# hyperlogic/splatapult

Measured on AMD Instinct MI355X. Metric: frames_per_sec, higher is better.
Workload: dtype f32; 1 GPU; 1M synthetic Gaussians, SH3, 1920x1080 fp32, 64-step orbit (BASELINE configs[1]); key=cfg2, splats=1000000, width=1920, height=1080, views=1, framebuffer=fp32, frames_in_flight=4, gpu_max_hw_queues=4, async_submit=True, cameras=64-step orbit

## Files before the change

### __graft_entry__.py

```python
import os
import subprocess
import sys

ROOT = os.path.dirname(os.path.abspath(__file__))
LIB = os.path.join(ROOT, "splatapult_amd", "lib", "libmsplat.so")
SOURCES = [os.path.join(ROOT, "splatapult_amd", "csrc", "msplat_device.hip"),
           os.path.join(ROOT, "splatapult_amd", "csrc", "msplat_group.hip"),
           os.path.join(ROOT, "splatapult_amd", "host", "gaussian_scene.cpp"),
           os.path.join(ROOT, "splatapult_amd", "host", "scene_config.cpp"),
           os.path.join(ROOT, "splatapult_amd", "host", "point_scene.cpp")]
HEADERS = [os.path.join(ROOT, "splatapult_amd", "csrc", h) for h in
           ("msplat_kernels.hip.h", "msplat_common.hip.h", "msplat_sort.hip.h", "msplat_cloud.hip.h", "msplat_project.hip.h",
            "msplat_binning.hip.h", "msplat_composite.hip.h", "msplat_points.hip.h", "msplat_occlusion.hip.h",
            "msplat_upload.hip.inc", "msplat_bands.hip.inc", "msplat_getters.hip.inc")] + [
           os.path.join(ROOT, "splatapult_amd", "host", "gaussian_scene.hpp"),
           os.path.join(ROOT, "splatapult_amd", "host", "scene_config.hpp"),
           os.path.join(ROOT, "splatapult_amd", "host", "point_scene.hpp"),
           os.path.join(ROOT, "splatapult_amd", "host", "two_pass_controller.hpp"),
           os.path.join(ROOT, "include", "msplat.h"), os.path.join(ROOT, "include", "msplat_debug.h")]
HIPCC_FLAGS = ["--offload-arch=gfx950", "-O3", "-std=c++17", "-fPIC", "-shared", "-ffp-contract=off",
               "-Wall", "-Wno-unused-function"]


def _stale(target, deps):
    if not os.path.exists(target):
        return True
    t = os.path.getmtime(target)
    return any(os.path.getmtime(d) > t for d in deps if os.path.exists(d))


def build(force=False):
    os.makedirs(os.path.dirname(LIB), exist_ok=True)
    if force or _stale(LIB, SOURCES + HEADERS):
        hipcc = os.environ.get("HIPCC", "/opt/rocm/bin/hipcc")
        cmd = [hipcc] + HIPCC_FLAGS + ["-o", LIB] + SOURCES + ["-lpthread"]
        subprocess.run(cmd, check=True, cwd=ROOT)
    subprocess.run(["make", "-C", os.path.join(ROOT, "oracle")], check=True, stdout=subprocess.DEVNULL)
    if ROOT not in sys.path:
        sys.path.insert(0, ROOT)
    import splatapult_amd
    L = splatapult_amd.lib()
    from splatapult_amd import _capi
    for name, _, _ in _capi.SYMBOLS:
        if os.environ.get("MSPLAT_LIB_PATH") and not hasattr(L, name):
            continue
        getattr(L, name)
# ... 37 lines not shown
```

### include/msplat_debug.h

```cpp
#ifndef MSPLAT_DEBUG_H
#define MSPLAT_DEBUG_H

#include "msplat.h"

#ifdef __cplusplus
extern "C" {
#endif

int msplat_debug_get_projected(msplat_ctx* ctx, float* rec12, uint32_t* rect, uint32_t cap);
int msplat_debug_get_tile_lists(msplat_ctx* ctx, uint32_t* tile_start, uint32_t tile_cap, uint32_t* pairs, uint64_t pair_cap);
int msplat_debug_verify_order(msplat_ctx* ctx, uint32_t* key_violations, uint32_t* list_violations);
int msplat_debug_get_cull_boxes(msplat_ctx* ctx, uint32_t* live, uint32_t* total, int* listed);

int msplat_debug_two_pass(msplat_ctx* ctx, float share, uint64_t* two_pass_frames, float* share_now);
int msplat_get_two_pass_info(msplat_ctx* ctx, uint64_t out[8]);

typedef struct msplat_composite_work {
    uint64_t work_items;
    uint64_t list_entries;
    uint64_t pair_words_fetched;
    uint64_t records_fetched;
    uint64_t records_composited;
    uint64_t pixel_evals;
    uint64_t batches;
    uint64_t clocks_sum, clocks_max, inner_clocks_sum;
    uint64_t useful_evals;
} msplat_composite_work;
int msplat_set_tile_probe(msplat_ctx* ctx, int enable);
int msplat_debug_get_tile_probe8(msplat_ctx* ctx, uint32_t* dst8, uint32_t tile_cap);
int msplat_get_composite_work(msplat_ctx* ctx, msplat_composite_work* out);

int msplat_debug_get_compositor_launch(msplat_ctx* ctx, uint32_t out[4]);

int msplat_debug_band_exchange_loopback(msplat_ctx* ctx, void* comm, int32_t kind, int32_t block_rows, int32_t world, int32_t rank,
                                        const void* src, void* dst, uint64_t pitch_bytes, int32_t width, int32_t height, int32_t flags);

int msplat_debug_cu_partition(msplat_ctx* ctx, uint32_t* mask8);

int msplat_debug_sh_q8_round(const float rec_in[61], float rec_out[61], float steps_out[3], int8_t codes_out[45]);

int msplat_debug_upload_kernel_ms(msplat_ctx* ctx, float* ms);

#ifdef __cplusplus
}
#endif
#endif
```

### splatapult_amd/_capi.py

```python
import ctypes as C
import os

_HERE = os.path.dirname(os.path.abspath(__file__))
LIB_PATH = os.environ.get("MSPLAT_LIB_PATH") or os.path.join(_HERE, "lib", "libmsplat.so")

OK = 0
ERR_INVALID_ARG, ERR_NO_DEVICE, ERR_HIP, ERR_NO_CLOUD, ERR_NO_SORT, ERR_UNSUPPORTED, ERR_PAIR_OVERFLOW, ERR_IO = \
    -1, -2, -3, -4, -5, -6, -7, -8
ERR_PAIR_OVERFLOW_EARLIER = -9
FB_RGBA32F, FB_RGBA16F, FB_RGBA8, FB_SRGB8_ALPHA8 = 0, 1, 2, 3
FB_FORMATS = {"fp32": FB_RGBA32F, "fp16": FB_RGBA16F, "rgba8": FB_RGBA8, "srgb8": FB_SRGB8_ALPHA8}
FB_NAMES = {v: n for n, v in FB_FORMATS.items()}
FB_DTYPES = {FB_RGBA32F: "float32", FB_RGBA16F: "float16", FB_RGBA8: "uint8", FB_SRGB8_ALPHA8: "uint8"}
ROP_NONE, ROP_RGBA8, ROP_RGBA16F = 0, 1, 2
RANK_AUTO, RANK_BALLOT = 0, 1
FRAMES_AUTO, FRAMES_SERIAL, FRAMES_IN_FLIGHT = 0, 1, 2
SPATIAL_AUTO, SPATIAL_ON, SPATIAL_OFF = 0, 1, 2
TWO_PASS_AUTO, TWO_PASS_ON, TWO_PASS_OFF = 0, 1, 2
BANDS_CONTIGUOUS, BANDS_INTERLEAVED, BANDS_BLOCK_INTERLEAVED, BANDS_ROOT_WEIGHTED = 0, 1, 2, 3
EXCHANGE_WIRE_FP16 = 1
CU_ALL, CU_EVEN, CU_ODD = 0, 1, 2
STORAGE_FP32, STORAGE_SH_FP16 = 0, 1
CLOUD_STORAGES = {"fp32": STORAGE_FP32, "sh_fp16": STORAGE_SH_FP16}
STORAGE_SH_Q8 = 3
# ... 112 lines not shown
    ("msplat_points_import_ply", C.c_int, [C.c_void_p, C.c_char_p]),
    ("msplat_points_export_ply", C.c_int, [C.c_void_p, C.c_char_p]),
    ("msplat_points_init_debug", None, [C.c_void_p]),
    ("msplat_points_num", C.c_uint64, [C.c_void_p]),
    ("msplat_points_stride", C.c_uint32, [C.c_void_p]),
    ("msplat_points_data", C.c_void_p, [C.c_void_p]),
    ("msplat_upload_points", C.c_int, [C.c_void_p, C.c_void_p, C.c_uint64, C.c_uint32, C.c_uint32, C.c_uint32]),
    ("msplat_upload_point_cloud", C.c_int, [C.c_void_p, C.c_void_p]),
    ("msplat_set_point_sprite", C.c_int, [C.c_void_p, C.c_void_p, C.c_uint32, C.c_uint32]),
    ("msplat_set_depth_test", C.c_int, [C.c_void_p, C.c_int]),
    ("msplat_set_target_emulation", C.c_int, [C.c_void_p, C.c_int]),
    ("msplat_set_target_mode", C.c_int, [C.c_void_p, C.c_int32]),
    ("msplat_get_target_mode", C.c_int, [C.c_void_p]),
    ("msplat_group_set_target_mode", C.c_int, [C.c_void_p, C.c_int32]),
    ("msplat_attach_cloud", C.c_int, [C.c_void_p, C.c_void_p]),
    ("msplat_stream_wait", C.c_int, [C.c_void_p, C.c_void_p]),
    ("msplat_wait_event", C.c_int, [C.c_void_p, C.c_void_p]),
    ("msplat_sort_count", C.c_int, [C.c_void_p, _U32P]),
    ("msplat_get_sorted_indices", C.c_int, [C.c_void_p, _U32P, C.c_uint32]),
    ("msplat_get_sorted_keys", C.c_int, [C.c_void_p, _U32P, C.c_uint32]),
    ("msplat_get_storage_order", C.c_int, [C.c_void_p, _U32P, C.c_uint64, C.POINTER(C.c_int)]),
    ("msplat_debug_get_cull_boxes", C.c_int, [C.c_void_p, _U32P, _U32P, C.POINTER(C.c_int)]),
    ("msplat_get_stats", C.c_int, [C.c_void_p, C.POINTER(Stats)]),
    ("msplat_get_timings", C.c_int, [C.c_void_p, C.POINTER(Timings)]),
    ("msplat_debug_get_projected", C.c_int, [C.c_void_p, _F16, _U32P, C.c_uint32]),
    ("msplat_debug_get_tile_lists", C.c_int, [C.c_void_p, _U32P, C.c_uint32, _U32P, C.c_uint64]),
    ("msplat_debug_get_tile_probe8", C.c_int, [C.c_void_p, _U32P, C.c_uint32]),
    ("msplat_set_tile_probe", C.c_int, [C.c_void_p, C.c_int]),
    ("msplat_debug_verify_order", C.c_int, [C.c_void_p, _U32P, _U32P]),
    ("msplat_debug_two_pass", C.c_int, [C.c_void_p, C.c_float, C.POINTER(C.c_uint64), C.POINTER(C.c_float)]),
    ("msplat_get_two_pass_info", C.c_int, [C.c_void_p, C.POINTER(C.c_uint64)]),
    ("msplat_get_composite_work", C.c_int, [C.c_void_p, C.POINTER(CompositeWork)]),
    ("msplat_debug_get_compositor_launch", C.c_int, [C.c_void_p, _U32P]),
    ("msplat_cloud_create", C.c_void_p, [C.c_int]),
    ("msplat_cloud_destroy", None, [C.c_void_p]),
    ("msplat_cloud_import_ply", C.c_int, [C.c_void_p, C.c_char_p]),
    ("msplat_cloud_export_ply", C.c_int, [C.c_void_p, C.c_char_p]),
    ("msplat_cloud_init_debug", C.c_int, [C.c_void_p]),
    ("msplat_cloud_prune", C.c_int, [C.c_void_p, _F16, C.c_uint32]),
    ("msplat_cloud_from_attributes", C.c_int, [C.c_void_p, C.c_uint64, _F16, _F16, _F16, _F16, _F16, _F16]),
    ("msplat_cloud_num_gaussians", C.c_uint64, [C.c_void_p]),
    ("msplat_cloud_stride", C.c_uint64, [C.c_void_p]),
    ("msplat_cloud_total_size", C.c_uint64, [C.c_void_p]),
    ("msplat_cloud_raw_data", C.c_void_p, [C.c_void_p]),
    ("msplat_cloud_has_full_sh", C.c_int, [C.c_void_p]),
    ("msplat_cloud_attr_offsets", C.c_int, [C.c_void_p, C.POINTER(AttrOffsets)]),
    ("msplat_upload_gaussian_cloud", C.c_int, [C.c_void_p, C.c_void_p]),
    ("msplat_cameras_import_json", C.c_int, [C.c_char_p, _F16, _F16, C.c_uint32, _U32P]),
    ("msplat_cameras_floor_plane", C.c_int, [C.c_char_p, _F16, _F16]),
    ("msplat_vrconfig_import_json", C.c_int, [C.c_char_p, _F16]),
    ("msplat_vrconfig_export_json", C.c_int, [C.c_char_p, _F16]),
    ("msplat_find_config_file", C.c_int, [C.c_char_p, C.c_char_p, C.c_char_p, C.c_uint32]),
    ("msplat_write_image", C.c_int, [C.c_char_p, _F16, C.c_int, C.c_int, C.c_int]),
    ("msplat_mat4_inverse", None, [_F16, _F16]),
    ("msplat_mat4_mul", None, [_F16, _F16, _F16]),
    ("msplat_perspective", None, [C.c_float, C.c_float, C.c_float, C.c_float, _F16]),
    ("msplat_create_projection", None, [C.c_float] * 6 + [_F16]),
]

_LIB = None


def lib():
    global _LIB
    if _LIB is None:
        if not os.path.exists(LIB_PATH):
# ... 70 lines not shown
```

### splatapult_amd/csrc/msplat_device.hip

```cpp
#include "msplat_kernels.hip.h"

#include <hip/hip_ext.h>

#include <algorithm>
#include <cmath>
#include <cstdarg>
#include <cstdio>
#include <cstdlib>
#include <cstring>
#include <exception>
#include <condition_variable>
#include <deque>
#include <functional>
#include <memory>
#include <mutex>
#include <thread>
#include <string>
#include <type_traits>
#include <vector>

#include "../../include/msplat.h"
#include "../../include/msplat_debug.h"
#include "../host/two_pass_controller.hpp"

using namespace msplat;

namespace {

thread_local std::string g_last_error;

struct Buf {
    void* p = nullptr;
    size_t bytes = 0;
    bool frame_table = false;
};

struct CloudStore {
    int device = 0;
    Buf pos4, recs;
    int storage = kStorageFp32;
    int F4 = 0;
    bool reordered = false;
    std::vector<uint32_t> order_host;
    Buf boxes;
    uint32_t nboxes = 0;
    ~CloudStore()
    {
        (void)hipSetDevice(device);
        if (pos4.p) (void)hipFree(pos4.p);
        if (recs.p) (void)hipFree(recs.p);
        if (boxes.p) (void)hipFree(boxes.p);
    }
};

inline uint32_t* words(const Buf& b) { return (uint32_t*)b.p; }

// ... 83 lines not shown
    HistTable hist;
    GroupTable gsumS[2];
    GroupTable gsumB1, gsumB2;
    WideSort ws;
    bool wide_sort_cfg = true;
    Buf vmask;
    Buf live_list, live_cnt;
    int spatial_mode = 0;
    bool last_sort_listed = false;
    FrameParams last_sort_fp{};
    uint32_t sort_parity = 0;
    bool tables_dirty = false;
    Buf bincnt;
    Buf heavy, heavy_flag;
    uint32_t render_parity = 0;
    bool scan_free = true;
    uint32_t grid_cap = kGridCap;
    Buf totals;
    Buf totals1;
    Buf counters;
    Buf queue;
    uint64_t rank_cap = 0;
    Buf rec2d;
    Buf rect;
    Buf zq;
    int depth_bits = 0;
    int rop = 0;
    int target_mode = MSPLAT_TARGET_CLEAR;
    bool point_mode = false;
    Buf sprite;
    SpriteParams sprite_params{};
    Buf tile_start;
    Buf tile_order;
    HistTable hist1;
    Buf pairsA, pairsB;
    uint64_t pair_cap = 0;
    HistTable hist2;
    Buf fb;
    Buf fbz;
    Buf fbo;
    Buf probe;
    bool probe_on = false;
    uint32_t* h_flags = nullptr;
    uint32_t* d_flags = nullptr;
    bool banded = false;
    int band_first = 0, band_block = 1, band_stride = 1, band_count = 0;
    bool band_cull = false;
    FrameParams last_fp{};
    bool has_render = false;
    static constexpr int kEvSets = 32;
    hipEvent_t ev[kEvSets][kEvSlots]{};
    bool ev_ok = false;
    int timing_stride = 1;
    uint64_t sort_calls = 0, render_calls = 0;
    uint32_t sort_sets = 0, render_sets = 0;
    int cur_render_set = -1;
    bool comp_kernel_timed = false;
    uint32_t comp_kernel_sets_mask = 0;
    uint32_t two_pass_sets_mask = 0;
    Buf occ, occ_mask, occ_fin, occ_state, occ_live, occ_boxdead, occ_unf;
    Buf occ_zstate;
    int two_pass_mode = MSPLAT_TWO_PASS_AUTO;
    TwoPassController two_pass;
    bool last_render_two_pass = false;
    uint32_t comp_launch[4] = {0, 0, 0, 0};
    uint64_t frames_two_pass = 0;
// ... 255 lines not shown
        if (c.cu_partition == MSPLAT_CU_EVEN || c.cu_partition == MSPLAT_CU_ODD) {
            hipDeviceProp_t prop;
            if (hipGetDeviceProperties(&prop, ctx->device) == hipSuccess && prop.multiProcessorCount == 256) {
                uint32_t mask[8] = {0};
                for (int i = 0; i < 256; ++i)
                    if ((i / 8) % 2 == c.cu_partition - MSPLAT_CU_EVEN) mask[i / 32] |= 1u << (i % 32);
                e = hipExtStreamCreateWithCUMask(&ctx->stream, 8, mask);
                ctx->cu_partition = e == hipSuccess ? c.cu_partition : MSPLAT_CU_ALL;
            }
            if (e != hipSuccess) (void)hipGetLastError();
        }
        if (e != hipSuccess) e = hipStreamCreateWithFlags(&ctx->stream, hipStreamNonBlocking);
        if (e != hipSuccess) {
            delete ctx;
            return fail(nullptr, MSPLAT_ERR_HIP, "hipStreamCreate: %s", hipGetErrorString(e));
        }
        ctx->own_stream = true;
    }
    if (c.enable_timing > 0) {
        bool ok = true;
        for (auto& set : ctx->ev)
            for (auto& ev : set) ok = ok && (hipEventCreate(&ev) == hipSuccess);
        ctx->ev_ok = ok;
        ctx->timing_stride = c.enable_timing;
    }
    int rc = buf_alloc(ctx, ctx->totals, 256 * sizeof(uint32_t));
    if (rc == MSPLAT_OK) rc = buf_alloc(ctx, ctx->counters, kCounterCount * sizeof(uint32_t));
    if (rc == MSPLAT_OK) rc = buf_alloc(ctx, ctx->totals1, 256 * sizeof(uint32_t));
    if (rc == MSPLAT_OK) rc = buf_alloc(ctx, ctx->queue, kQueueShards * kQueueStride * sizeof(uint32_t));
    ctx->queue.frame_table = ctx->bincnt.frame_table = true;
    if (rc == MSPLAT_OK) rc = buf_alloc(ctx, ctx->tile_start, (65536 + 1024 + 16) * sizeof(uint32_t));
    if (rc == MSPLAT_OK) rc = buf_alloc(ctx, ctx->bincnt, (65536 + 1024 + 16) * sizeof(uint32_t));
    if (rc == MSPLAT_OK && hipMemsetAsync(ctx->bincnt.p, 0, ctx->bincnt.bytes, ctx->stream) != hipSuccess) rc = MSPLAT_ERR_HIP;
    if (rc == MSPLAT_OK) rc = buf_alloc(ctx, ctx->tile_order, 2 * 65536 * sizeof(uint32_t));

    if (c.compositor_waves > 0) { ctx->comp_waves = std::max(64, (int)c.compositor_waves); ctx->comp_waves_auto = false; }
    if (rc == MSPLAT_OK) {
        if (hipHostMalloc((void**)&ctx->h_flags, kHostWordCount * sizeof(uint32_t), hipHostMallocMapped) != hipSuccess ||
            hipHostGetDevicePointer((void**)&ctx->d_flags, ctx->h_flags, 0) != hipSuccess)
            rc = fail(ctx, MSPLAT_ERR_HIP, "msplat_create: cannot allocate the host-mapped status words");
        else
            std::memset(ctx->h_flags, 0, kHostWordCount * sizeof(uint32_t));
    }
    if (rc == MSPLAT_OK && hipMemsetAsync(ctx->counters.p, 0, kCounterCount * sizeof(uint32_t), ctx->stream) != hipSuccess)
        rc = MSPLAT_ERR_HIP;
    if (rc == MSPLAT_OK && hipMemsetAsync((uint32_t*)ctx->counters.p + kCntMinKey, 0xFF, 2 * sizeof(uint32_t), ctx->stream) != hipSuccess)
        rc = MSPLAT_ERR_HIP;
    if (rc == MSPLAT_OK) {
        uint32_t* bad = (uint32_t*)ctx->counters.p + kCntLdsProbe;
        hipLaunchKernelGGL(iota_kernel, dim3(65536 / kThreads), dim3(kThreads), 0, ctx->stream, (uint32_t*)ctx->tile_order.p + 65536);
        hipLaunchKernelGGL(lds_atomic_order_probe, dim3(64), dim3(kThreads), 0, ctx->stream, bad);
        uint32_t hbad = 1;
        if (hipMemcpyAsync(&hbad, bad, sizeof(hbad), hipMemcpyDeviceToHost, ctx->stream) != hipSuccess ||
            hipStreamSynchronize(ctx->stream) != hipSuccess)
            rc = fail(ctx, MSPLAT_ERR_HIP, "LDS atomic order probe failed to run");
        ctx->atomic_rank = (hbad == 0) && c.rank_mode != MSPLAT_RANK_BALLOT;
        ctx->scan_free = getenv("MSPLAT_SCAN_KERNELS") == nullptr;
        ctx->ws.threads = c.frame_mode == MSPLAT_FRAMES_IN_FLIGHT ? (uint32_t)kWsThreadsSmall : (uint32_t)kWsThreads;
        if (const char* sk = getenv("MSPLAT_SORT")) ctx->wide_sort_cfg = std::string(sk) != "lsd8";
        if (const char* gc = getenv("MSPLAT_GRID_CAP")) ctx->grid_cap = (uint32_t)std::min(std::max(atol(gc), 1L), (long)kGridCap);
        if (!ctx->atomic_rank) ctx->wide_sort_cfg = false;
        ctx->spatial_mode = c.spatial_order;
        if (ctx->wide_sort_cfg) {
            static std::mutex lds_mu;
            static int lds_state[64];
            const int dslot = ctx->device & 63;
            std::lock_guard<std::mutex> lk(lds_mu);
// ... 21 lines not shown
            AsyncWorker* w = ctx->worker.get();
            const msplat_ctx* self = ctx;
            const int dev = ctx->device;
            w->th = std::thread([w, self, dev] {
                (void)hipSetDevice(dev);
                g_on_worker_of = self;
                w->run();
            });
        } catch (const std::exception&) {
            ctx->worker.reset();
        }
    }
    *out = ctx;
    return MSPLAT_OK;
}

void msplat_destroy(msplat_ctx* ctx)
{
    if (!ctx) return;
    if (ctx->worker) {
        ctx->worker->drain();
        { std::lock_guard<std::mutex> lk(ctx->worker->mu); ctx->worker->quit = true; }
        ctx->worker->cv.notify_all();
        if (ctx->worker->th.joinable()) ctx->worker->th.join();
        ctx->worker.reset();
    }
    (void)hipSetDevice(ctx->device);
    (void)hipStreamSynchronize(ctx->stream);
    ctx->pos4 = Buf{};
    ctx->recs = Buf{};
    ctx->store.reset();
    if (ctx->join_ev) (void)hipEventDestroy(ctx->join_ev);
    if (ctx->h_flags) (void)hipHostFree(ctx->h_flags);
    for (Buf* b : ctx->bufs) buf_free(ctx, *b);
    if (ctx->ev_ok)
        for (auto& set : ctx->ev)
            for (auto& ev : set) (void)hipEventDestroy(ev);
    if (ctx->own_stream) (void)hipStreamDestroy(ctx->stream);
    delete ctx;
}

static int ensure_pair_capacity(msplat_ctx* ctx, uint64_t cap);

static int poll_async_overflow(msplat_ctx* ctx, std::string& msg)
{
    uint32_t need = host_word(ctx, kHostOverflowPairs);
    if (need == 0) return MSPLAT_OK;
    if (hipSetDevice(ctx->device) != hipSuccess || hipStreamSynchronize(ctx->stream) != hipSuccess)
        return fail(ctx, MSPLAT_ERR_HIP, "hipStreamSynchronize failed while handling a pair-buffer overflow");
    need = std::max(need, host_word(ctx, kHostOverflowPairs));
    __atomic_store_n(ctx->h_flags + kHostOverflowPairs, 0u, __ATOMIC_RELAXED);
    const uint64_t old_cap = ctx->pair_cap;
    char buf[384];
    if (ctx->cfg.pair_capacity == 0 && (uint64_t)need + (need >> 2) + 1024 <= 0x7FFFFFFFull &&
        ensure_pair_capacity(ctx, (uint64_t)need + (need >> 2) + 1024) == MSPLAT_OK) {
        snprintf(buf, sizeof(buf), "an earlier device-output render overflowed the pair buffer (needed %u pairs, capacity "
                 "was %llu): that frame lacks splats in its last bin columns; capacity grown to %llu", need,
                 (unsigned long long)old_cap, (unsigned long long)ctx->pair_cap);
    } else {
        snprintf(buf, sizeof(buf), "an earlier device-output render overflowed the pair buffer (needed %u pairs, capacity "
                 "%llu%s): that frame lacks splats in its last bin columns", need, (unsigned long long)old_cap,
                 ctx->cfg.pair_capacity ? ", fixed by msplat_config.pair_capacity" : "");
    }
    msg = buf;
    return MSPLAT_ERR_PAIR_OVERFLOW;
}
// ... 562 lines not shown
                       keep_overflow, d_first);
    if (!fused1)
        launch_scan(s, small, ctx->hist1, d_V, 0u, N, bchunk, totals1);
    with_flag(ctx->atomic_rank, [&](auto AR) {
        hipLaunchKernelGGL((bin1_downsweep<AR.value, kBinChunk>), dim3(g1 + nhelp), dim3(kThreads), 0, s,
                           (const uint32_t*)ctx->rect.p, d_V, (const uint32_t*)words(ctx->hist1.buf), ctx->hist1.stride,
                           (const uint32_t*)totals1, (uint32_t*)ctx->pairsA.p, cap, d_D, d_overflow, ctx->d_flags,
                           async_overflow_flag ? 1 : 0, fused1 ? (const uint32_t*)gB1 : nullptr, fused1 ? totals1 : nullptr,
                           xcdg, (const uint32_t*)hv_cur, (const uint8_t*)ctx->heavy_flag.p,
                           (uint32_t)nhelp, fp.tiles_x, ctx->gsumB1.sup, (const uint32_t*)d_Vsort,
                           (keep_overflow && ctx->d_flags) ? ctx->d_flags + kHostPass2Pairs : (uint32_t*)nullptr, ctx->two_pass.seq, d_first);
    });
    const bool wave_comp = !draw_order_frame(ctx);
    const uint32_t comp_items = (uint32_t)ntiles * 4u;
    const uint32_t comp_pool = (ctx->comp_waves_auto && comp_items <= (stereo ? 40960u : 20480u)) ? comp_items : (uint32_t)ctx->comp_waves;
    const bool ordered = !(wave_comp && comp_pool < comp_items);
    const int g2 = grid_for(div_up(cap, kPairChunk), ctx->grid_cap);
    RadixPass a;
    a.keys_in = (const uint32_t*)ctx->pairsA.p;  a.keys_out = (uint32_t*)ctx->pairsB.p;
    a.d_n = d_D;  a.n_cap = cap;  a.shift = 24;  a.fp = &fp;
    a.hist = &ctx->hist2;  a.totals = totals2;  a.totals_out = fused2 ? totals2 : nullptr;
    a.gsum = &ctx->gsumB2;  a.gsum_zero = &ctx->gsumB1;  a.fused = fused2;
    a.col_totals = totals1;  a.bincnt = (uint32_t*)ctx->bincnt.p;  a.queue = d_queue;
    a.tile_start = (uint32_t*)ctx->tile_start.p;  a.tile_order = (uint32_t*)ctx->tile_order.p;  a.ntiles = ntiles;  a.do_order = (ordered ? 1 : 0) | 2;
    launch_radix_upsweep<MODE_PAIR, kSortItems, true>(s, g2, a);
    if (!fused2)
        launch_scan(s, small, ctx->hist2, d_D, 0u, cap, (uint32_t)kPairChunk, totals2);
    with_flag(ctx->atomic_rank, [&](auto AR) { launch_radix_downsweep<MODE_PAIR, false, AR.value, kSortItems, true>(s, g2 + 1, a); });
    rc.ordered = ordered;
    rc.comp_items = comp_items;
    rc.comp_pool = comp_pool;
}

static int issue_compositor(RenderChain& rc, int occ_pass, int ev_c0, int ev_c1)
{
    msplat_ctx* ctx = rc.ctx;
    const FrameParams& fp = rc.fp;
    hipStream_t s = rc.s;
    const uint32_t cap = rc.cap, comp_items = rc.comp_items, comp_pool = rc.comp_pool;
    const bool stereo = rc.stereo, timed = rc.timed, ordered = rc.ordered;
    const int ntiles = rc.ntiles, tset = rc.tset;
    uint32_t *d_queue = rc.d_queue, *occ = rc.occ;
    void *d_out = rc.d_out, *d_out1 = rc.d_out1;
    const size_t pitch = rc.pitch;
    uint32_t* fin = occ_pass ? (uint32_t*)ctx->occ_fin.p : nullptr;
    float4* state = occ_pass ? (float4*)ctx->occ_state.p : nullptr;
    const uint32_t* d_nbins = occ_pass == 2 ? occ + kOccUnfinished : nullptr;
    const FramePlanes& pl = rc.planes;
    const bool draw_order = draw_order_frame(ctx);
    auto with_format = [&](auto&& f) { with_int<kFbF16, kFbUnorm8, kFbSrgb8, kFbF32>(ctx->cfg.fb_format, f); };

    const int cgrid = std::min(ntiles * 4, ctx->comp_waves);
    if (ntiles > 0 && occ_pass != 2) {
        ctx->comp_launch[0] = draw_order ? (uint32_t)ntiles * 4u : comp_items;
        ctx->comp_launch[1] = draw_order ? (uint32_t)cgrid : std::min(comp_items, comp_pool);
        ctx->comp_launch[2] = ordered ? 1u : 0u;
        ctx->comp_launch[3] = ctx->point_mode ? 2u : draw_order ? 1u : 0u;
    }
    if (ntiles > 0 && ctx->probe_on && ctx->probe.p && draw_order)
        HIP_TRY(ctx, hipMemsetAsync(ctx->probe.p, 0, (size_t)ntiles * 8 * kProbeWords * sizeof(uint32_t), s));
    if (ntiles > 0 && ctx->point_mode) {
        const uint32_t* zqp = ctx->depth_bits ? (const uint32_t*)ctx->zq.p : nullptr;
        with_format([&](auto FMT) {
            hipLaunchKernelGGL(composite_points_kernel<FMT.value>, dim3(cgrid), dim3(kCompThreads), 0, s,
                               (const uint32_t*)ctx->tile_start.p, (const uint32_t*)ctx->pairsB.p,
                               (const float4*)ctx->rec2d.p, zqp, (const float4*)ctx->sprite.p, ctx->sprite_params, d_out,
                               pitch, fp, cap, (const uint32_t*)ctx->tile_order.p, d_queue, (uint32_t)ntiles * 4u);
        });
        ctx->comp_kernel_timed = false;
    } else if (ntiles > 0 && draw_order) {
        with_format([&](auto FMT) {
            with_int<kTargetLoad, kTargetPremultiplied, kTargetClear>(ctx->target_mode, [&](auto TM) {
                hipLaunchKernelGGL((composite_depth_kernel<FMT.value, TM.value>), dim3(cgrid), dim3(kCompThreads), 0, s,
                                   (const uint32_t*)ctx->tile_start.p, (const uint32_t*)ctx->pairsB.p,
                                   (const float4*)ctx->rec2d.p, (const uint32_t*)ctx->zq.p, d_out, pitch, fp, cap,
                                   (const uint32_t*)ctx->tile_order.p, d_queue, (uint32_t)ntiles * 4u);
            });
        });
        ctx->comp_kernel_timed = false;
    } else if (ntiles > 0) {
        hipEvent_t e0 = timed ? ctx->ev[tset][ev_c0] : nullptr, e1 = timed ? ctx->ev[tset][ev_c1] : nullptr;
        uint32_t* probe = ctx->probe_on ? (uint32_t*)ctx->probe.p : nullptr;
        if (probe) HIP_TRY(ctx, hipMemsetAsync(probe, 0, (size_t)ntiles * 8 * kProbeWords * sizeof(uint32_t), s));
        const uint32_t* ts = (const uint32_t*)ctx->tile_start.p;
        const uint32_t* pb = (const uint32_t*)ctx->pairsB.p;
        const float4* r2 = (const float4*)ctx->rec2d.p;
        const uint32_t* ord = occ_pass == 2 ? (const uint32_t*)ctx->occ_unf.p : (const uint32_t*)ctx->tile_order.p + (ordered ? 0 : 65536);
        const int prio_mode = ordered ? 1 : 0;
        const int grid = (int)std::min<uint32_t>(comp_items, comp_pool);
        const CompParams cp = comp_params(fp);
        const CompExtra ex{d_out1, fin, state, d_nbins, probe, (const float*)ctx->zq.p, pl.depth[0], pl.depth_pitch,
                           occ_pass ? (float*)ctx->occ_zstate.p : nullptr, pl.occluder[0], pl.occluder_pitch, pl.occluder[1], pl.depth[1]};
        const int prio = occ_pass == 2 ? 0 : prio_mode;
        auto composite = [&](auto OCC, auto TWO, auto PROBE, auto TM, auto DEPTH, auto ZTEST) {
            with_format([&](auto FMT) {
                hipExtLaunchKernelGGL((composite_kernel<FMT.value, OCC.value, TWO.value, PROBE.value, TM.value, DEPTH.value, ZTEST.value>),
                                      dim3(grid), dim3(kCompThreads), 0, s, e0, e1, 0, ts, pb, r2, d_out, pitch, cp, cap, ord, d_queue,
                                      comp_items, prio, ex);
            });
        };
        constexpr flag_t<true> yes{};
        constexpr flag_t<false> no{};
        auto form = [&](auto OCC, auto TWO) {
            with_int<kTargetLoad, kTargetPremultiplied, kTargetClear>(ctx->target_mode, [&](auto TM) {
                if constexpr (OCC.value == 0 && TM.value == kTargetClear) {
                    if (probe && !pl.any()) return composite(OCC, TWO, yes, TM, no, no);
                }
                with_flag(!!pl.depth[0], [&](auto DEPTH) {
                    with_flag(!!pl.occluder[0], [&](auto ZTEST) { composite(OCC, TWO, no, TM, DEPTH, ZTEST); });
                });
            });
        };
        if (stereo) form(int_t<0>{}, yes);
        else with_int<1, 2, 0>(occ_pass, [&](auto OCC) { form(OCC, no); });
        ctx->comp_kernel_timed = timed;
    } else {
        ctx->comp_kernel_timed = false;
    }
    return MSPLAT_OK;
}
// ... 335 lines not shown
```

### splatapult_amd/csrc/msplat_getters.hip.inc

```

#ifdef MSPLAT_STAMPS
static msplat::StampRec* g_stamps_dev = nullptr;
static uint32_t g_stamps_slots = 0;
int msplat_debug_stamps(int enable, uint32_t log2_slots)
{
    if (enable && !g_stamps_dev) {
        g_stamps_slots = 1u << std::min(26u, std::max(10u, log2_slots));
        if (hipMalloc((void**)&g_stamps_dev, (size_t)g_stamps_slots * sizeof(msplat::StampRec)) != hipSuccess) return MSPLAT_ERR_HIP;
        if (hipMemset(g_stamps_dev, 0, (size_t)g_stamps_slots * sizeof(msplat::StampRec)) != hipSuccess) return MSPLAT_ERR_HIP;
        if (hipMemcpyToSymbol(HIP_SYMBOL(msplat::g_stamp_buf), &g_stamps_dev, sizeof(g_stamps_dev)) != hipSuccess) return MSPLAT_ERR_HIP;
    }
    if (hipDeviceSynchronize() != hipSuccess) return MSPLAT_ERR_HIP;
    const uint32_t mask = (enable && g_stamps_dev) ? g_stamps_slots - 1u : 0u;
    if (hipMemcpyToSymbol(HIP_SYMBOL(msplat::g_stamp_mask), &mask, sizeof(mask)) != hipSuccess) return MSPLAT_ERR_HIP;
    return hipDeviceSynchronize() == hipSuccess ? (int)g_stamps_slots : MSPLAT_ERR_HIP;
}
int msplat_debug_stamps_read(void* dst, uint64_t bytes)
{
    if (!g_stamps_dev || !dst) return MSPLAT_ERR_INVALID_ARG;
    const size_t n = std::min<size_t>(bytes, (size_t)g_stamps_slots * sizeof(msplat::StampRec));
    if (hipDeviceSynchronize() != hipSuccess || hipMemcpy(dst, g_stamps_dev, n, hipMemcpyDeviceToHost) != hipSuccess) return MSPLAT_ERR_HIP;
    if (hipMemset(g_stamps_dev, 0, (size_t)g_stamps_slots * sizeof(msplat::StampRec)) != hipSuccess) return MSPLAT_ERR_HIP;
    return MSPLAT_OK;
}
// ... 256 lines not shown
        h.resize((size_t)items * kProbeWords);
    } catch (const std::exception&) {
        return fail(ctx, MSPLAT_ERR_HIP, "out of host memory");
    }
    int rc = msplat_debug_get_tile_probe8(ctx, h.data(), items);
    if (rc) return rc;
    for (uint32_t t = 0; t < items; ++t) {
        const uint32_t* p = &h[(size_t)t * kProbeWords];
        if (!p[7]) continue;
        out->work_items += 1;
        out->clocks_sum += p[0];
        out->clocks_max = std::max<uint64_t>(out->clocks_max, p[0]);
        out->records_composited += p[1];
        out->pixel_evals += (uint64_t)p[1] * (uint64_t)(kTile * kTile);
        out->batches += p[2];
        out->inner_clocks_sum += p[3];
        out->pair_words_fetched += p[4];
        out->records_fetched += p[5];
        out->list_entries += p[6];
        out->useful_evals += (uint64_t)(p[7] - 1u);
    }
    return MSPLAT_OK;
}

int msplat_debug_get_compositor_launch(msplat_ctx* ctx, uint32_t out[4])
{
    drain_async(ctx);
    if (!ctx || !out) return fail(ctx, MSPLAT_ERR_INVALID_ARG, "NULL argument");
    if (!ctx->has_render) return fail(ctx, MSPLAT_ERR_NO_SORT, "no render yet");
    for (int i = 0; i < 4; ++i) out[i] = ctx->comp_launch[i];
    return MSPLAT_OK;
}

int msplat_debug_get_tile_lists(msplat_ctx* ctx, uint32_t* tile_start, uint32_t tile_cap,
                                uint32_t* pairs, uint64_t pair_cap)
{
    drain_async(ctx);
    if (!ctx) return fail(nullptr, MSPLAT_ERR_INVALID_ARG, "ctx is NULL");
    if (!ctx->has_render) return fail(ctx, MSPLAT_ERR_NO_SORT, "no render yet");
    HIP_TRY(ctx, hipSetDevice(ctx->device));
    HIP_TRY(ctx, hipStreamSynchronize(ctx->stream));
    const uint32_t ntiles = (uint32_t)(ctx->last_fp.tiles_x * ctx->last_fp.tiles_y);
    if (tile_cap < ntiles + 1) return fail(ctx, MSPLAT_ERR_INVALID_ARG, "tile capacity too small");
    if (tile_start) HIP_TRY(ctx, hipMemcpy(tile_start, ctx->tile_start.p, (size_t)(ntiles + 1) * 4, hipMemcpyDeviceToHost));
    uint32_t cnt[4];
    HIP_TRY(ctx, hipMemcpy(cnt, ctx->counters.p, sizeof(cnt), hipMemcpyDeviceToHost));
    const uint64_t d = std::min<uint64_t>(cnt[kCntD], ctx->pair_cap);
    if (pairs) {
        if (pair_cap < d) return fail(ctx, MSPLAT_ERR_INVALID_ARG, "pair capacity too small");
        if (d) HIP_TRY(ctx, hipMemcpy(pairs, ctx->pairsB.p, d * 4, hipMemcpyDeviceToHost));
    }
    return MSPLAT_OK;
}

int msplat_debug_cu_partition(msplat_ctx* ctx, uint32_t* mask8)
{
    if (!ctx) return MSPLAT_ERR_INVALID_ARG;
    if (mask8) {
        memset(mask8, 0, 8 * sizeof(uint32_t));
        if (hipSetDevice(ctx->device) != hipSuccess || hipExtStreamGetCUMask(ctx->stream, 8, mask8) != hipSuccess) {
            (void)hipGetLastError();
            return fail(ctx, MSPLAT_ERR_HIP, "msplat_debug_cu_partition: hipExtStreamGetCUMask failed");
        }
    }
    return ctx->cu_partition;
}
// ... 8 lines not shown
```

### splatapult_amd/renderer.py

```python
import ctypes as C

import numpy as np

from . import _capi
from .scene import GaussianCloud


class _FrameArgs:
    __slots__ = ("buf", "cam", "proj", "vp", "nf", "p_cam", "p_proj", "p_vp", "p_nf")

    def __init__(self):
        self.buf = np.zeros(38, np.float32)
        self.cam, self.proj, self.vp, self.nf = self.buf[0:16], self.buf[16:32], self.buf[32:36], self.buf[36:38]
        base = self.buf.ctypes.data
        fp = C.POINTER(C.c_float)
        self.p_cam, self.p_proj = C.cast(base, fp), C.cast(base + 64, fp)
        self.p_vp, self.p_nf = C.cast(base + 128, fp), C.cast(base + 144, fp)

    @staticmethod
    def _flat(a, n):
        a = np.asarray(a, np.float32).reshape(-1)
        if a.shape[0] != n:
            raise AssertionError("expected %d floats" % n)
        return a
# ... 449 lines not shown
            t = _capi.Timings()
            _capi.check(h, self._lib.msplat_get_timings(h, C.byref(t)))
            nf = t.reserved[0]
            frames += nf
            for k in keys:
                acc[k] += getattr(t, k) * nf
            acc["composite_kernel"] += t.reserved[1] * nf
        d = {k: (v / frames if frames > 0 else 0.0) for k, v in acc.items()}
        d["frames_averaged"] = frames
        return d

    def debug_projected(self):
        v = self.sort_count()
        rec = np.zeros((max(v, 1), 12), np.float32)
        rect = np.zeros(max(v, 1), np.uint32)
        _capi.check(self._ctx, self._lib.msplat_debug_get_projected(
            self._ctx, rec.ctypes.data_as(C.POINTER(C.c_float)), rect.ctypes.data_as(C.POINTER(C.c_uint32)), rec.shape[0]))
        return rec[:v], rect[:v]

    def set_tile_probe(self, enable=True):
        for h in self._ctxs:
            _capi.check(h, self._lib.msplat_set_tile_probe(h, 1 if enable else 0))

    def composite_work(self):
        w = _capi.CompositeWork()
        _capi.check(self._ctx, self._lib.msplat_get_composite_work(self._ctx, C.byref(w)))
        return {k: int(getattr(w, k)) for k, _ in _capi.CompositeWork._fields_}

    def compositor_launch(self):
        out = (C.c_uint32 * 4)()
        _capi.check(self._ctx, self._lib.msplat_debug_get_compositor_launch(self._ctx, out))
        return tuple(int(v) for v in out)

    def two_pass_state(self, share=0.0):
        frames, now = 0, 0.0
        for h in self._ctxs:
            a, b = C.c_uint64(), C.c_float()
            _capi.check(h, self._lib.msplat_debug_two_pass(h, float(share), C.byref(a), C.byref(b)))
            frames += a.value
            now = b.value
        return frames, now

    def two_pass_info(self):
        out = (C.c_uint64 * 8)()
        _capi.check(self._ctx, self._lib.msplat_get_two_pass_info(self._ctx, out))
        if out[0] == 0:
            return None
        keys = ("frames", "splats_pass1", "splats_pass2", "pairs_pass1", "pairs_pass2", "bins_unfinished", "bins", "visible")
        return {k: int(out[i]) for i, k in enumerate(keys)}

    def verify_order(self):
        a, b = C.c_uint32(), C.c_uint32()
        _capi.check(self._ctx, self._lib.msplat_debug_verify_order(self._ctx, C.byref(a), C.byref(b)))
        return a.value, b.value

    def cu_partitions(self):
        out = []
        for h in self._ctxs:
            m = (C.c_uint32 * 8)()
            rc = self._lib.msplat_debug_cu_partition(h, m)
            _capi.check(h, rc if rc < 0 else 0)
            out.append((rc, list(m)))
        return out

    def debug_tile_probe(self):
        st = self.stats()
# ... 135 lines not shown
```

Before: 6731 frames/s.

## Order unordered compositor bins in XCD-aware 4x4 tile blocks

Adds a host-computed bin order for the unordered compositor path. Tiles are grouped into 4x4 blocks and blocks are dealt round-robin across the 8 XCDs, so workgroups landing on the same XCD handle spatially nearby tiles and can share L2 hits on splat records. The order is computed once per resolution, uploaded asynchronously into a third slot of tile_order, and replaces the previous unordered order. It assumes the hardware dispatches workgroups round-robin across XCDs, and it adds debug getters for inspecting the order.

```diff
diff --git a/__graft_entry__.py b/__graft_entry__.py
--- a/__graft_entry__.py
+++ b/__graft_entry__.py
@@ -11,7 +11,7 @@
            os.path.join(ROOT, "splatapult_amd", "host", "point_scene.cpp")]
 HEADERS = [os.path.join(ROOT, "splatapult_amd", "csrc", h) for h in
            ("msplat_kernels.hip.h", "msplat_common.hip.h", "msplat_sort.hip.h", "msplat_cloud.hip.h", "msplat_project.hip.h",
-            "msplat_binning.hip.h", "msplat_composite.hip.h", "msplat_points.hip.h", "msplat_occlusion.hip.h",
+            "msplat_binning.hip.h", "msplat_composite.hip.h", "msplat_points.hip.h", "msplat_occlusion.hip.h", "msplat_bin_order.h",
             "msplat_upload.hip.inc", "msplat_bands.hip.inc", "msplat_getters.hip.inc")] + [
            os.path.join(ROOT, "splatapult_amd", "host", "gaussian_scene.hpp"),
            os.path.join(ROOT, "splatapult_amd", "host", "scene_config.hpp"),
diff --git a/include/msplat_debug.h b/include/msplat_debug.h
--- a/include/msplat_debug.h
+++ b/include/msplat_debug.h
@@ -32,6 +32,9 @@
 
 int msplat_debug_get_compositor_launch(msplat_ctx* ctx, uint32_t out[4]);
 
+int msplat_debug_bin_order(int32_t tiles_x, int32_t rows, uint32_t* out);
+int msplat_debug_get_bin_order(msplat_ctx* ctx, uint32_t* out, uint32_t cap);
+
 int msplat_debug_band_exchange_loopback(msplat_ctx* ctx, void* comm, int32_t kind, int32_t block_rows, int32_t world, int32_t rank,
                                         const void* src, void* dst, uint64_t pitch_bytes, int32_t width, int32_t height, int32_t flags);
 
diff --git a/splatapult_amd/_capi.py b/splatapult_amd/_capi.py
--- a/splatapult_amd/_capi.py
+++ b/splatapult_amd/_capi.py
@@ -168,6 +168,8 @@
     ("msplat_get_two_pass_info", C.c_int, [C.c_void_p, C.POINTER(C.c_uint64)]),
     ("msplat_get_composite_work", C.c_int, [C.c_void_p, C.POINTER(CompositeWork)]),
     ("msplat_debug_get_compositor_launch", C.c_int, [C.c_void_p, _U32P]),
+    ("msplat_debug_bin_order", C.c_int, [C.c_int32, C.c_int32, _U32P]),
+    ("msplat_debug_get_bin_order", C.c_int, [C.c_void_p, _U32P, C.c_uint32]),
     ("msplat_cloud_create", C.c_void_p, [C.c_int]),
     ("msplat_cloud_destroy", None, [C.c_void_p]),
     ("msplat_cloud_import_ply", C.c_int, [C.c_void_p, C.c_char_p]),
diff --git a/splatapult_amd/csrc/msplat_bin_order.h b/splatapult_amd/csrc/msplat_bin_order.h
--- /dev/null
+++ b/splatapult_amd/csrc/msplat_bin_order.h
@@ -0,0 +1,35 @@
+#pragma once
+
+#include <stdint.h>
+
+#include <vector>
+
+namespace msplat {
+
+constexpr int kXcds = 8;
+constexpr int kBinBlockW = 4, kBinBlockH = 4;
+
+inline void bin_order_xcd(int tiles_x, int rows, int bw, int bh, uint32_t* out)
+{
+    std::vector<uint32_t> cls[kXcds];
+    const int nbx = (tiles_x + bw - 1) / bw, nby = (rows + bh - 1) / bh;
+    for (int by = 0; by < nby; ++by)
+        for (int bx = 0; bx < nbx; ++bx) {
+            std::vector<uint32_t>& c = cls[(by * nbx + bx) % kXcds];
+            for (int y = by * bh; y < rows && y < (by + 1) * bh; ++y)
+                for (int x = bx * bw; x < tiles_x && x < (bx + 1) * bw; ++x) c.push_back((uint32_t)(y * tiles_x + x));
+        }
+    size_t next[kXcds] = {0, 0, 0, 0, 0, 0, 0, 0};
+    const int nbins = tiles_x * rows;
+    for (int s = 0; s < nbins; ++s) {
+        int c = s % kXcds;
+        if (next[c] == cls[c].size()) {
+            size_t most = 0;
+            for (int k = 0; k < kXcds; ++k)
+                if (cls[k].size() - next[k] > most) { most = cls[k].size() - next[k]; c = k; }
+        }
+        out[s] = cls[c][next[c]++];
+    }
+}
+
+}
diff --git a/splatapult_amd/csrc/msplat_device.hip b/splatapult_amd/csrc/msplat_device.hip
--- a/splatapult_amd/csrc/msplat_device.hip
+++ b/splatapult_amd/csrc/msplat_device.hip
@@ -22,6 +22,7 @@
 #include "../../include/msplat.h"
 #include "../../include/msplat_debug.h"
 #include "../host/two_pass_controller.hpp"
+#include "msplat_bin_order.h"
 
 using namespace msplat;
 
@@ -171,6 +172,11 @@
     SpriteParams sprite_params{};
     Buf tile_start;
     Buf tile_order;
+    int bin_order_tx = 0, bin_order_rows = 0;
+    uint32_t* bin_order_host = nullptr;
+    hipEvent_t bin_order_ev = nullptr;
+    const uint32_t* comp_order = nullptr;
+    uint32_t comp_order_bins = 0;
     HistTable hist1;
     Buf pairsA, pairsB;
     uint64_t pair_cap = 0;
@@ -492,7 +498,7 @@
     if (rc == MSPLAT_OK) rc = buf_alloc(ctx, ctx->tile_start, (65536 + 1024 + 16) * sizeof(uint32_t));
     if (rc == MSPLAT_OK) rc = buf_alloc(ctx, ctx->bincnt, (65536 + 1024 + 16) * sizeof(uint32_t));
     if (rc == MSPLAT_OK && hipMemsetAsync(ctx->bincnt.p, 0, ctx->bincnt.bytes, ctx->stream) != hipSuccess) rc = MSPLAT_ERR_HIP;
-    if (rc == MSPLAT_OK) rc = buf_alloc(ctx, ctx->tile_order, 2 * 65536 * sizeof(uint32_t));
+    if (rc == MSPLAT_OK) rc = buf_alloc(ctx, ctx->tile_order, 3 * 65536 * sizeof(uint32_t));
 
     if (c.compositor_waves > 0) { ctx->comp_waves = std::max(64, (int)c.compositor_waves); ctx->comp_waves_auto = false; }
     if (rc == MSPLAT_OK) {
@@ -580,6 +586,8 @@
     ctx->store.reset();
     if (ctx->join_ev) (void)hipEventDestroy(ctx->join_ev);
     if (ctx->h_flags) (void)hipHostFree(ctx->h_flags);
+    if (ctx->bin_order_host) (void)hipHostFree(ctx->bin_order_host);
+    if (ctx->bin_order_ev) (void)hipEventDestroy(ctx->bin_order_ev);
     for (Buf* b : ctx->bufs) buf_free(ctx, *b);
     if (ctx->ev_ok)
         for (auto& set : ctx->ev)
@@ -1208,6 +1216,25 @@
     rc.comp_pool = comp_pool;
 }
 
+static int ensure_bin_order(msplat_ctx* ctx, int tiles_x, int rows, hipStream_t s)
+{
+    if (ctx->bin_order_tx == tiles_x && ctx->bin_order_rows == rows) return MSPLAT_OK;
+    if (!ctx->bin_order_host) {
+        HIP_TRY(ctx, hipHostMalloc((void**)&ctx->bin_order_host, 65536 * sizeof(uint32_t), hipHostMallocDefault));
+        HIP_TRY(ctx, hipEventCreateWithFlags(&ctx->bin_order_ev, hipEventDisableTiming));
+    } else {
+        HIP_TRY(ctx, hipEventSynchronize(ctx->bin_order_ev));
+    }
+    bin_order_xcd(tiles_x, rows, kBinBlockW, kBinBlockH, ctx->bin_order_host);
+    ctx->bin_order_tx = ctx->bin_order_rows = 0;
+    HIP_TRY(ctx, hipMemcpyAsync((uint32_t*)ctx->tile_order.p + 2 * 65536, ctx->bin_order_host, (size_t)tiles_x * rows * sizeof(uint32_t),
+                                hipMemcpyHostToDevice, s));
+    HIP_TRY(ctx, hipEventRecord(ctx->bin_order_ev, s));
+    ctx->bin_order_tx = tiles_x;
+    ctx->bin_order_rows = rows;
+    return MSPLAT_OK;
+}
+
 static int issue_compositor(RenderChain& rc, int occ_pass, int ev_c0, int ev_c1)
 {
     msplat_ctx* ctx = rc.ctx;
@@ -1232,6 +1259,8 @@
         ctx->comp_launch[1] = draw_order ? (uint32_t)cgrid : std::min(comp_items, comp_pool);
         ctx->comp_launch[2] = ordered ? 1u : 0u;
         ctx->comp_launch[3] = ctx->point_mode ? 2u : draw_order ? 1u : 0u;
+        ctx->comp_order = (const uint32_t*)ctx->tile_order.p;
+        ctx->comp_order_bins = (uint32_t)ntiles;
     }
     if (ntiles > 0 && ctx->probe_on && ctx->probe.p && draw_order)
         HIP_TRY(ctx, hipMemsetAsync(ctx->probe.p, 0, (size_t)ntiles * 8 * kProbeWords * sizeof(uint32_t), s));
@@ -1261,7 +1290,14 @@
         const uint32_t* ts = (const uint32_t*)ctx->tile_start.p;
         const uint32_t* pb = (const uint32_t*)ctx->pairsB.p;
         const float4* r2 = (const float4*)ctx->rec2d.p;
-        const uint32_t* ord = occ_pass == 2 ? (const uint32_t*)ctx->occ_unf.p : (const uint32_t*)ctx->tile_order.p + (ordered ? 0 : 65536);
+        const bool xcd_order = !ordered && occ_pass != 2 && !probe;
+        if (xcd_order) {
+            const int rc_order = ensure_bin_order(ctx, fp.tiles_x, fp.tiles_y, s);
+            if (rc_order != MSPLAT_OK) return rc_order;
+        }
+        const uint32_t* ord = occ_pass == 2 ? (const uint32_t*)ctx->occ_unf.p
+                                            : (const uint32_t*)ctx->tile_order.p + (ordered ? 0 : xcd_order ? 2 * 65536 : 65536);
+        if (occ_pass != 2) { ctx->comp_order = ord; ctx->comp_order_bins = (uint32_t)ntiles; }
         const int prio_mode = ordered ? 1 : 0;
         const int grid = (int)std::min<uint32_t>(comp_items, comp_pool);
         const CompParams cp = comp_params(fp);
diff --git a/splatapult_amd/csrc/msplat_getters.hip.inc b/splatapult_amd/csrc/msplat_getters.hip.inc
--- a/splatapult_amd/csrc/msplat_getters.hip.inc
+++ b/splatapult_amd/csrc/msplat_getters.hip.inc
@@ -312,6 +312,25 @@
     return MSPLAT_OK;
 }
 
+int msplat_debug_get_bin_order(msplat_ctx* ctx, uint32_t* out, uint32_t cap)
+{
+    drain_async(ctx);
+    if (!ctx || !out) return fail(ctx, MSPLAT_ERR_INVALID_ARG, "NULL argument");
+    if (!ctx->has_render || !ctx->comp_order) return fail(ctx, MSPLAT_ERR_NO_SORT, "no render yet");
+    if (cap < ctx->comp_order_bins) return fail(ctx, MSPLAT_ERR_INVALID_ARG, "capacity %u < %u bins", cap, ctx->comp_order_bins);
+    HIP_TRY(ctx, hipSetDevice(ctx->device));
+    HIP_TRY(ctx, hipStreamSynchronize(ctx->stream));
+    HIP_TRY(ctx, hipMemcpy(out, ctx->comp_order, (size_t)ctx->comp_order_bins * sizeof(uint32_t), hipMemcpyDeviceToHost));
+    return MSPLAT_OK;
+}
+
+int msplat_debug_bin_order(int32_t tiles_x, int32_t rows, uint32_t* out)
+{
+    if (!out || tiles_x < 1 || rows < 1 || tiles_x > 256 || rows > 256) return MSPLAT_ERR_INVALID_ARG;
+    bin_order_xcd(tiles_x, rows, kBinBlockW, kBinBlockH, out);
+    return MSPLAT_OK;
+}
+
 int msplat_debug_get_tile_lists(msplat_ctx* ctx, uint32_t* tile_start, uint32_t tile_cap,
                                 uint32_t* pairs, uint64_t pair_cap)
 {
diff --git a/splatapult_amd/renderer.py b/splatapult_amd/renderer.py
--- a/splatapult_amd/renderer.py
+++ b/splatapult_amd/renderer.py
@@ -505,6 +505,11 @@
         _capi.check(self._ctx, self._lib.msplat_debug_get_compositor_launch(self._ctx, out))
         return tuple(int(v) for v in out)
 
+    def bin_order(self):
+        out = np.zeros(max(self.compositor_launch()[0] // 4, 1), np.uint32)
+        _capi.check(self._ctx, self._lib.msplat_debug_get_bin_order(self._ctx, out.ctypes.data_as(C.POINTER(C.c_uint32)), out.shape[0]))
+        return out
+
     def two_pass_state(self, share=0.0):
         frames, now = 0, 0.0
         for h in self._ctxs:
```

Result: faster. 6871 frames/s (median of 6 runs) (+2.1%).
